# datastax/jvector

Measured on AMD Instinct MI355X. Metric: QPS@recall10>=0.95 (10Mx768); distances/sec as % HBM roofline, higher is better.
Workload: dtype f32

## Files before the change

### jvector_amd/csrc/cabi.cpp

```cpp
#include <algorithm>
#include <cmath>
#include <cstring>
#include <mutex>

#include "jv_device.h"
#include "jv_internal.h"
#include "gs_params.h"
#include "../../include/jvector_formats.h"

namespace jv {

static thread_local char g_err[1024] = "";

void set_error(const char *fmt, ...)
{
    va_list ap;
    va_start(ap, fmt);
    vsnprintf(g_err, sizeof(g_err), fmt, ap);
    va_end(ap);
}
void clear_error() { g_err[0] = 0; }

int Buffer::reserve(size_t bytes)
{
// ... 188 lines not shown
    int n = jv_hip_device_count();
    if (n <= 0) {
        set_error("no HIP device visible (libjvector_hip has no CPU fallback)");
        return JV_ERR_NO_DEVICE;
    }
    JV_REQUIRE(device >= 0 && device < n, "ctx_create: device %d out of range [0,%d)", device, n);
    JV_TRY(use_device(device));
    hipDeviceProp_t prop;
    JV_HIP_CHECK(hipGetDeviceProperties(&prop, device));
    if (strncmp(prop.gcnArchName, "gfx950", 6) != 0) {
        set_error("device %d is %s; this library contains gfx950 code objects only", device, prop.gcnArchName);
        return JV_ERR_NO_DEVICE;
    }
    jv_ctx *c = new jv_ctx();
    c->device = device;
    c->num_cus = prop.multiProcessorCount;
    c->lds_per_block = prop.maxSharedMemoryPerMultiProcessor ? (size_t)prop.maxSharedMemoryPerMultiProcessor
                                                             : (size_t)prop.sharedMemPerBlock;
    if (c->lds_per_block > 160 * 1024) c->lds_per_block = 160 * 1024;
    if (stream != JV_STREAM_PRIVATE) {
        c->stream = (hipStream_t)stream;
        c->owns_stream = false;
    } else {
        hipError_t e = hipStreamCreateWithFlags(&c->stream, hipStreamNonBlocking);
        if (e != hipSuccess) {
            set_error("hipStreamCreate failed: %s", hipGetErrorString(e));
            delete c;
            return JV_ERR_HIP;
        }
        c->owns_stream = true;
    }
    c->h_in.pinned_host = true;
    c->h_out.pinned_host = true;
    *out = c;
    return JV_OK;
}

int jv_hip_ctx_destroy(jv_ctx *ctx)
{
    if (!ctx) return JV_OK;
    (void)hipSetDevice(ctx->device);
    (void)hipStreamSynchronize(ctx->stream);
    if (ctx->host_pool && ctx->host_pool_destroy) ctx->host_pool_destroy(ctx->host_pool);
    ctx->h_in.release();
    ctx->h_out.release();
    ctx->d_in.release();
    ctx->d_out.release();
    ctx->d_scratch.release();
    ctx->d_scratch2.release();
    ctx->d_scratch3.release();
    ctx->d_gs_visited.release();
    ctx->d_gs_spill.release();
    ctx->d_gs_out.release();
    ctx->d_gs_mask.release();
    ctx->d_gs_big.release();
    ctx->d_nvq_q.release();
    ctx->d_gs_extra.release();
    ctx->d_gs_ubr.release();
    ctx->d_bq_work.release();
    ctx->d_bin_work.release();
    ctx->d_bin_cand.release();
    ctx->d_rd_counts.release();
    for (auto &e : ctx->prof_pending) {
        (void)hipEventDestroy(e.start);
        (void)hipEventDestroy(e.stop);
    }
    for (auto &e : ctx->prof_free) (void)hipEventDestroy(e);
    if (ctx->owns_stream) (void)hipStreamDestroy(ctx->stream);
    delete ctx;
    return JV_OK;
}

int jv_hip_ctx_sync(jv_ctx *ctx)
{
    JV_REQUIRE(ctx, "ctx is NULL");
    JV_HIP_CHECK(hipStreamSynchronize(ctx->stream));
    return JV_OK;
}
// ... 615 lines not shown
    l->device = ctx->device;
    l->pq = pq;
    l->capacity = max_queries;
    auto fail = [&](hipError_t e) {
        set_error("luts_create: hipMalloc failed: %s", hipGetErrorString(e));
        (void)hipGetLastError();
        jv_hip_luts_destroy(l);
        return JV_ERR_OOM;
    };
    hipError_t e;
    if ((e = hipMalloc((void **)&l->d_luts, sizeof(float) * (size_t)max_queries * pq->M * kClusters)) != hipSuccess) return fail(e);
    if ((e = hipMalloc((void **)&l->d_bmag, sizeof(float) * (size_t)max_queries)) != hipSuccess) return fail(e);
    if ((e = hipMalloc((void **)&l->d_queries, sizeof(float) * (size_t)max_queries * pq->D)) != hipSuccess) return fail(e);
    if ((e = hipMalloc((void **)&l->d_raw_queries, sizeof(float) * (size_t)max_queries * pq->D)) != hipSuccess) return fail(e);
    *out = l;
    return JV_OK;
}

int jv_hip_luts_destroy(jv_luts *l)
{
    if (!l) return JV_OK;
    (void)hipSetDevice(l->device);
    (void)hipFree(l->d_luts);
    (void)hipFree(l->d_bmag);
    (void)hipFree(l->d_queries);
    (void)hipFree(l->d_raw_queries);
    delete l;
    return JV_OK;
}

}

namespace jv {
int luts_prepare(jv_ctx *ctx, jv_luts *l, const float *queries, int Q, jv_vsf vsf, jv_decoder_kind kind, bool with_tables)
{
    JV_REQUIRE(ctx && l, "luts_build: NULL argument");
    JV_REQUIRE(Q >= 0 && Q <= l->capacity, "luts_build: Q=%d exceeds capacity %d", Q, l->capacity);
    JV_REQUIRE(vsf == JV_EUCLIDEAN || vsf == JV_DOT_PRODUCT || vsf == JV_COSINE, "Unsupported similarity function %d",
               (int)vsf);
    l->Q = Q;
    l->vsf = vsf;
    l->kind = kind;
    l->tables_valid = false;
    if (Q == 0) return JV_OK;
    JV_REQUIRE(queries, "luts_build: queries is NULL");
    JV_TRY(use_device(ctx->device));
    const jv_pq *pq = l->pq;
    const size_t qbytes = sizeof(float) * (size_t)Q * pq->D;
    if (is_device_ptr(queries)) {
        JV_HIP_CHECK(hipMemcpyAsync(l->d_raw_queries, queries, qbytes, hipMemcpyDeviceToDevice, ctx->stream));
    } else {
        JV_HIP_CHECK(hipStreamSynchronize(ctx->stream));
        JV_TRY(ctx->h_in.reserve(qbytes));
        memcpy(ctx->h_in.ptr, queries, qbytes);
        JV_HIP_CHECK(hipMemcpyAsync(l->d_raw_queries, ctx->h_in.ptr, qbytes, hipMemcpyHostToDevice, ctx->stream));
    }
    ProfScope ps(ctx, R_LUT);
    JV_TRY(launch_center_queries(ctx->stream, pq, l->d_raw_queries, Q, l->d_queries));
    if (with_tables) {
        const int lut_vsf = (vsf == JV_EUCLIDEAN) ? VSF_L2 : VSF_DOT;
        JV_TRY(launch_lut_build(ctx->stream, pq, l->d_queries, Q, lut_vsf, l->d_luts));
        l->tables_valid = true;
    }
    if (vsf == JV_COSINE)
        JV_TRY(launch_query_magnitudes(ctx->stream, pq, l->d_queries, Q, kind == JV_DECODER_FUSED ? 1 : 0, l->d_bmag));
    return JV_OK;
}
}

extern "C" {

int jv_hip_luts_build(jv_ctx *ctx, jv_luts *l, const float *queries, int Q, jv_vsf vsf, jv_decoder_kind kind)
{
    clear_error();
    return luts_prepare(ctx, l, queries, Q, vsf, kind, true);
}

int jv_hip_luts_download(jv_ctx *ctx, const jv_luts *l, int q, float *lut_out, float *bmag_out)
{
    clear_error();
    JV_REQUIRE(ctx && l, "luts_download: NULL argument");
    JV_REQUIRE(q >= 0 && q < l->Q, "luts_download: query %d out of range", q);
    JV_REQUIRE(l->tables_valid || !lut_out, "luts_download: the tables were overwritten by a table-free graph search; call jv_hip_luts_build again");
    JV_TRY(use_device(ctx->device));
    JV_HIP_CHECK(hipStreamSynchronize(ctx->stream));
    const size_t n = (size_t)l->pq->M * kClusters;
    if (lut_out) JV_HIP_CHECK(hipMemcpy(lut_out, l->d_luts + (size_t)q * n, sizeof(float) * n, hipMemcpyDefault));
    if (bmag_out) {
        if (l->vsf == JV_COSINE) JV_HIP_CHECK(hipMemcpy(bmag_out, l->d_bmag + q, sizeof(float), hipMemcpyDefault));
        else *bmag_out = 0.0f;
    }
// ... 264 lines not shown
    JV_TRY(ctx->d_scratch.reserve(topk_scratch_bytes(Q, k)));
    OutStage oi, osc;
    JV_TRY(stage_out_begin(ctx, out_ids, sizeof(int32_t) * (size_t)Q * k, ctx->d_out, &oi));
    JV_TRY(stage_out_begin(ctx, out_scores, sizeof(float) * (size_t)Q * k, ctx->d_scratch3, &osc));
    {
        ProfScope ps(ctx, R_TOPK);
        JV_TRY(launch_topk(ctx->stream, ctx, (const float *)d_scores, (const int32_t *)d_ids, Q, n, stride, id_base, k,
                           (int32_t *)oi.dev, (float *)osc.dev, ctx->d_scratch.ptr));
    }
    JV_TRY(stage_out_end(ctx, oi));
    return stage_out_end(ctx, osc);
}

static int next_pow2_i64(int64_t v)
{
    int64_t p = 1;
    while (p < v) p <<= 1;
    return (int)p;
}

int jv_hip_search_flat(jv_ctx *ctx, jv_luts *l, const jv_codes *codes, const jv_vectors *vectors, const float *queries,
                       int Q, jv_vsf vsf, int topK, int rerankK, int32_t id_base, int32_t *out_ids, float *out_scores)
{
    clear_error();
    JV_REQUIRE(ctx && l && codes, "search_flat: NULL argument");
    JV_REQUIRE(topK > 0, "search_flat: topK must be positive");
    const bool rerank = vectors != nullptr && rerankK > 0;
    JV_REQUIRE(!rerank || rerankK >= topK, "rerankK %d must be >= topK %d", rerankK, topK);
    JV_REQUIRE(!rerank || vectors->D == l->pq->D, "search_flat: vector dimension mismatch");
    JV_REQUIRE(!rerank || vectors->count >= codes->count, "search_flat: fewer vectors than codes");
    if (Q == 0) return JV_OK;
    JV_REQUIRE(out_ids && out_scores, "search_flat: NULL output");
    JV_TRY(use_device(ctx->device));
    JV_TRY(jv_hip_luts_build(ctx, l, queries, Q, vsf, JV_DECODER_PQ));
    if (vsf == JV_COSINE) JV_TRY(ensure_code_norms(ctx, const_cast<jv_codes *>(codes)));
    const int64_t N = codes->count;
    const int kvsf = to_kernel_vsf(vsf);
    const int k1 = rerank ? rerankK : topK;

    OutStage oi, osc;
    JV_TRY(stage_out_begin(ctx, out_ids, sizeof(int32_t) * (size_t)Q * topK, ctx->d_out, &oi));
    JV_TRY(stage_out_begin(ctx, out_scores, sizeof(float) * (size_t)Q * topK, ctx->d_in, &osc));

    const size_t c1 = (size_t)Q * k1;
    JV_TRY(ctx->d_scratch3.reserve(sizeof(int32_t) * c1 + sizeof(float) * c1 * 2 + sizeof(float) * (size_t)Q + 1024));
    int32_t *d_cand = (int32_t *)ctx->d_scratch3.ptr;
    float *d_cand_sc = (float *)(d_cand + c1);
    float *d_exact = d_cand_sc + c1;
    float *d_qnorm = d_exact + c1;
    int32_t *d_k1_ids = rerank ? d_cand : (int32_t *)oi.dev;
    float *d_k1_sc = rerank ? d_cand_sc : (float *)osc.dev;

    bool done1 = false;
    const bool mq = adc_mq_supported(codes->M, codes->d_codes) && Q >= 2;
    if (mq && N >= (1 << 18) && (int64_t)k1 * 64 <= N && ctx_opt(ctx, "no_filter", 0) == 0) {
        const int64_t c_target = std::max<int64_t>(3 * (int64_t)k1, 4096);
        int64_t S_target = std::max<int64_t>(16384, next_pow2_i64(32 * N / c_target));
        const int64_t stride = std::max<int64_t>(1, N / S_target);
        const int64_t S = N / stride;
        const int k_s = (int)std::max<int64_t>(16, (c_target * S + N - 1) / N);
        const int cap = (int)std::min<int64_t>(N, 4 * c_target);
        if (k_s <= 4096 && S >= k_s) {
            const size_t b_samp = sizeof(float) * (size_t)Q * S, b_ks = sizeof(float) * (size_t)Q * k_s;
            const size_t b_cap = sizeof(float) * (size_t)Q * cap;
            JV_TRY(ctx->d_scratch2.reserve(b_samp + 2 * b_ks + 2 * b_cap + sizeof(unsigned int) * (size_t)Q + 1024));
            char *base = (char *)ctx->d_scratch2.ptr;
            float *d_samp = (float *)base;
// ... 67 lines not shown
            JV_HIP_CHECK(hipMemcpyAsync(ctx->h_out.ptr, d_cnt, sizeof(unsigned int) * (size_t)Q, hipMemcpyDeviceToHost,
                                        ctx->stream));
            JV_HIP_CHECK(hipStreamSynchronize(ctx->stream));
            const unsigned int *cnt = (const unsigned int *)ctx->h_out.ptr;
            bool ok = true;
            for (int q = 0; q < Q; ++q) ok = ok && cnt[q] >= (unsigned int)k1 && cnt[q] <= (unsigned int)cap;
            if (ok) {
                ProfScope ps(ctx, R_TOPK);
                JV_TRY(launch_topk(ctx->stream, ctx, d_f_sc, d_f_ids, Q, cap, cap, 0, k1, d_k1_ids, d_k1_sc,
                                   ctx->d_scratch.ptr, d_cnt));
                done1 = true;
            }
            }
        }
    }
    if (!done1) {
        JV_TRY(ctx->d_scratch2.reserve(sizeof(float) * (size_t)Q * N));
        float *d_scores = (float *)ctx->d_scratch2.ptr;
        JV_TRY(ctx->d_scratch.reserve(topk_scratch_bytes(Q, std::max(k1, topK))));
        {
            ProfScope ps(ctx, R_ADC);
            if (mq)
                JV_TRY(launch_adc_mq_store(ctx->stream, ctx, l->d_luts, l->d_bmag, Q, codes->M, kvsf, codes->d_codes,
                                           codes->d_norms, 0, N, 1, d_scores));
            else
                JV_TRY(launch_adc(ctx->stream, ctx, l->d_luts, l->d_bmag, Q, codes->M, kvsf, codes->d_codes,
                                  codes->d_norms, N, 0, N, nullptr, d_scores));
        }
        ProfScope ps(ctx, R_TOPK);
        JV_TRY(launch_topk(ctx->stream, ctx, d_scores, nullptr, Q, N, N, 0, k1, d_k1_ids, d_k1_sc, ctx->d_scratch.ptr));
    }

    if (rerank) {
        JV_TRY(rerank_gather(ctx, vectors, l->d_raw_queries, Q, vsf, d_cand, k1, d_exact, d_qnorm));
        ProfScope ps(ctx, R_TOPK);
        JV_TRY(launch_topk(ctx->stream, ctx, d_exact, d_cand, Q, k1, k1, 0, topK, (int32_t *)oi.dev, (float *)osc.dev,
                           ctx->d_scratch.ptr));
    }
    JV_TRY(launch_add_id_base(ctx->stream, (int32_t *)oi.dev, (int64_t)Q * topK, id_base));
    JV_TRY(stage_out_end(ctx, oi));
    return stage_out_end(ctx, osc);
}

}
```

### jvector_amd/csrc/graph_search.cpp

```cpp
#include <algorithm>
#include <atomic>
#include <chrono>
#include <condition_variable>
#include <cstdlib>
#include <functional>
#include <memory>
#include <unordered_map>
#include <mutex>
#include <thread>

#include "gs_host.h"
#include "gs_params.h"
#include "jv_internal.h"

namespace jv {
constexpr long long kGsUbrDefault = 1;
constexpr long long kGsUbrcDefault = 1;


class HostPool {
public:
    explicit HostPool(int nthreads) : n_(nthreads)
    {
        for (int t = 1; t < n_; ++t) threads_.emplace_back([this, t] { worker(t); });
// ... 1161 lines not shown
    out->max_degree = 0;
    for (int l = 0; l <= g->entry_level; ++l) {
        const jv_graph::DevLevel &d = g->dev[l];
        lv[l].nbrs = d.nbrs;
        lv[l].hkeys = d.hkeys;
        lv[l].hvals = d.hvals;
        lv[l].hmask = d.hmask;
        lv[l].hshift = d.hshift;
        lv[l].count = g->levels[l].count;
        lv[l].degree = g->levels[l].degree;
        out->max_degree = std::max(out->max_degree, g->levels[l].degree);
    }
    return JV_OK;
}
}
}

struct DeviceSessionOut {
    float threshold = 0.0f;
    const std::vector<jv_searcher::Call> *history = nullptr;
    int new_rerankK = 0;
    int log_cap = 0;
    std::vector<int32_t> status, base, log_n;
    std::vector<int64_t> stats;
    std::vector<long long> log;
};

static int graph_search_device(jv_ctx *ctx, const jv_graph *g, jv_luts *l, const jv_codes *codes, const jv_fused *fused,
                               const jv_vectors *vectors, const float *queries, int Q, jv_vsf vsf, int topK, int rerankK,
                               int32_t *out_ids, float *out_scores, int64_t *stats, AcceptMask host_accept, AcceptMask dev_accept,
                               DeviceSessionOut *so = nullptr)
{
    const jv_decoder_kind kind = fused ? JV_DECODER_FUSED : JV_DECODER_PQ;
    JV_TRY(luts_prepare(ctx, l, queries, Q, vsf, kind, false));
    const int kvsf = to_kernel_vsf(vsf);
    if (vsf == JV_COSINE) {
        JV_TRY(ensure_code_norms(ctx, const_cast<jv_codes *>(codes)));
        if (fused) JV_TRY(ensure_fused_norms(ctx, const_cast<jv_fused *>(fused)));
    }
    JV_TRY(ensure_device_graph(ctx, const_cast<jv_graph *>(g)));
    const jv_pq *pq = l->pq;

    const bool generic = !graph_search_device_specialised(pq, codes, fused) || ctx_opt(ctx, "gs_generic", 0) != 0;
    const int occ = ctx_opt(ctx, "gs_occ", generic ? 4 : 2) >= 4 ? 4 : 2;
    bool pair = occ == 2 && !generic && ctx_opt(ctx, "gs_pair", 1) != 0;
    for (int lv = 0; lv <= g->entry_level; ++lv) pair = pair && g->levels[lv].degree <= 32;
    pair = pair && pq->M <= 96;
    const long long wgx_opt = ctx_opt(ctx, "gs_wgx", -1);
    bool one_wave_tuned = false;
    for (const char *o : {"gs_vcap_log2", "gs_v1_log2", "gs_grow", "gs_retry", "gs_occ", "gs_pair", "gs_cand_cap", "gs_waves_per_cu", "gs_prefetch", "gs_prof"})
        one_wave_tuned = one_wave_tuned || ctx_opt_is_set(ctx, o);
    bool wgx = !so && !generic && graph_search_wgx_supported(pq->M) &&
               (wgx_opt > 0 || (wgx_opt < 0 && !one_wave_tuned && Q <= 4 * ctx->num_cus));
    for (int lv = 0; lv <= g->entry_level; ++lv) wgx = wgx && g->levels[lv].degree <= 64;
    const int wgx_log = std::min(512, std::max(256, 4 * rerankK));
    int wgx_kps = 32;
    for (int lv = 0; lv <= g->entry_level; ++lv)
        if (g->levels[lv].degree > 32) wgx_kps = 64;
    const int wgx_waves = std::max(2, std::min(8, (int)ctx_opt(ctx, "gs_wgx_waves", 8)));
    const int wgx_slots = std::max(2, std::min((int)GX_MAX_SLOTS, (int)ctx_opt(ctx, "gs_wgx_slots", 16)));
    int evict_cap = GS_EVICT_CAP;
    const int wgx_cand_cap = 256;
    const int wgx_per_cu = std::max(1, std::min(4, (int)ctx_opt(ctx, "gs_wgx_per_cu", 1)));
    const size_t wgx_budget = ctx->lds_per_block / (size_t)wgx_per_cu - (wgx_per_cu > 1 ? 256 : 512);
    auto wgx_bytes = [&](int lg, int lm) { return graph_search_wgx_lds_bytes(pq->D, rerankK, wgx_cand_cap, evict_cap, lg, wgx_slots, wgx_kps, wgx_log, lm); };
    int wgx_lut_m = (int)ctx_opt(ctx, "gs_wgx_lut_m", 0);
    if (wgx) {
// ... 233 lines not shown
        p.big_visited = (int32_t *)ctx->d_gs_big.ptr;
        p.big_spill = (long long *)((char *)ctx->d_gs_big.ptr + big_spill_off);
        p.big_next = (uint32_t *)((char *)ctx->d_gs_big.ptr + big_ctr_off);
        p.big_count = big_count;
        p.big_log2 = big_log2;
        p.big_spill_cap = big_spill_cap;
    }
    p.pair = pair ? 1 : (pairc ? 2 : 0);
#ifdef JV_EXPERIMENTAL
    p.quad = ctx_opt(ctx, "gs_quad", 0) != 0 ? 1 : 0;
#else
    p.quad = 0;
#endif
    p.out_ids = d_cand;
    p.out_scores = d_cand_sc;
    p.out_stats = d_stats;
    p.out_status = d_status;
    p.next_query = d_counter;
    if (log_cap > 0) {
        p.push_log = (long long *)(base + o_log);
        p.push_log_n = (int32_t *)(base + o_log_n);
        p.push_log_cap = log_cap;
    }
    p.prof = gs_prof ? (unsigned long long *)(base + o_prof) : nullptr;
    p.plain = ctx_opt(ctx, "gs_plain", 1) != 0 ? 1 : 0;
    if (defer_on) {
        p.defer = 1;
        p.defer_count = (unsigned long long *)(base + o_prof) + 33;
        p.defer_min_level = (int)std::max<long long>(1, ctx_opt(ctx, "gs_defer_min_level", 2));
    }
    int rr_rows = 0;
    if (!so && !wgx && ubr && pair && vectors && !vectors->nvq && vectors->D == pq->D && gs_rr_lds_bytes() <= lds && ctx_opt(ctx, "gs_fused_rerank", 1) != 0) {
        if (vsf == JV_COSINE) JV_TRY(ensure_vector_norms(ctx, const_cast<jv_vectors *>(vectors)));
        rr_rows = exact_fused_rows(vectors->d_vecs, vectors->D, l->d_raw_queries, Q, kvsf, rerankK, vectors->d_sqnorm);
    }
    if (rr_rows > 0) {
        if (vsf == JV_COSINE) {
            ProfScope ps(ctx, R_EXACT);
            JV_TRY(launch_query_sqnorms(ctx->stream, l->d_raw_queries, vectors->D, Q, d_qnorm));
        }
        p.rr_vecs = vectors->d_vecs;
        p.rr_queries = l->d_raw_queries;
        p.rr_qnorm = d_qnorm;
        p.rr_vnorm = vectors->d_sqnorm;
        p.rr_n = vectors->count;
        p.rr_rows = rr_rows;
    }
    {
        ProfScope ps(ctx, R_GSEARCH);
        JV_TRY(launch(p, workers));
    }
    std::vector<int32_t> status((size_t)Q);
    std::vector<int> redo;
    size_t n_overflow_first = 0;
    {
        JV_TRY(ctx->h_out.reserve(sizeof(int32_t) * (size_t)Q));
        JV_HIP_CHECK(hipMemcpyAsync(ctx->h_out.ptr, d_status, sizeof(int32_t) * (size_t)Q, hipMemcpyDeviceToHost, ctx->stream));
        unsigned long long ubr_dropped = 0;
        if (ubr) JV_HIP_CHECK(hipMemcpyAsync(&ubr_dropped, base + o_prof + 15 * sizeof(unsigned long long), sizeof(ubr_dropped), hipMemcpyDeviceToHost, ctx->stream));
        unsigned long long defer_counts[3] = {0, 0, 0};
        if (defer_on) JV_HIP_CHECK(hipMemcpyAsync(defer_counts, base + o_prof + 33 * sizeof(unsigned long long), sizeof(defer_counts), hipMemcpyDeviceToHost, ctx->stream));
        JV_HIP_CHECK(hipStreamSynchronize(ctx->stream));
        if (ubr) ctx_stat_add(ctx, "gs_ubr_dropped", (long long)ubr_dropped);
        if (defer_on) {
            ctx_stat_add(ctx, "gs_deferred", (long long)defer_counts[0]);
            ctx_stat_add(ctx, "gs_defer_restarts", (long long)defer_counts[1]);
            if (Q >= 64 && defer_counts[1] * 10 > (unsigned long long)Q && g->defer_off.exchange(1, std::memory_order_relaxed) == 0)
                ctx_stat_add(ctx, "gs_defer_switched_off", 1);
        }
        memcpy(status.data(), ctx->h_out.ptr, sizeof(int32_t) * (size_t)Q);
        for (int q = 0; q < Q; ++q)
            if (status[q] != GS_OK) redo.push_back(q);
        n_overflow_first = redo.size();
    }
    const bool retry = ctx_opt_is_set(ctx, "gs_retry") ? ctx_opt(ctx, "gs_retry", 1) != 0 : !ctx_opt_is_set(ctx, "gs_vcap_log2");
    for (int attempt = 1; attempt <= 2 && !redo.empty() && retry; ++attempt) {
        const int vlog2 = std::min(24, vcap_log2 + 3 * attempt);
        if (vlog2 <= vcap_log2 + 3 * (attempt - 1)) break;
        const size_t vcap2 = (size_t)1 << vlog2;
        const int spill2 = (int)(vcap2 / 2 + v1_slots) + 64;
        const int R = (int)redo.size();
        const int workers2 = std::max(1, std::min<int>({R, workers, (int)(((size_t)512 << 20) / (vcap2 * 12))}));
        JV_TRY(ctx->d_gs_visited.reserve(sizeof(int32_t) * vcap2 * (size_t)workers2));
        JV_TRY(ctx->d_gs_spill.reserve(sizeof(long long) * (size_t)spill2 * (size_t)workers2));
        memcpy(ctx->h_out.ptr, redo.data(), sizeof(int32_t) * (size_t)R);
        JV_HIP_CHECK(hipMemcpyAsync(base + o_qmap, ctx->h_out.ptr, sizeof(int32_t) * (size_t)R, hipMemcpyHostToDevice, ctx->stream));
        JV_HIP_CHECK(hipMemsetAsync(d_counter, 0, sizeof(uint32_t), ctx->stream));
        GsParams p2 = p;
        p2.qmap = (const int32_t *)(base + o_qmap);
        p2.Q = R;
        p2.visited = (int32_t *)ctx->d_gs_visited.ptr;
        p2.vcap_log2 = vlog2;
        p2.spill = (long long *)ctx->d_gs_spill.ptr;
        p2.spill_cap = spill2;
        p2.big_visited = nullptr;
        p2.big_count = 0;
        p2.big_log2 = 0;
        p2.prof = nullptr;
        p2.defer = 0;
        {
            ProfScope ps(ctx, R_GSEARCH);
            JV_TRY(launch(p2, workers2));
        }
        JV_HIP_CHECK(hipStreamSynchronize(ctx->stream));
        JV_HIP_CHECK(hipMemcpyAsync(ctx->h_out.ptr, d_status, sizeof(int32_t) * (size_t)Q, hipMemcpyDeviceToHost, ctx->stream));
        JV_HIP_CHECK(hipStreamSynchronize(ctx->stream));
        memcpy(status.data(), ctx->h_out.ptr, sizeof(int32_t) * (size_t)Q);
        std::vector<int> still;
        for (int q : redo)
            if (status[q] != GS_OK) still.push_back(q);
        redo.swap(still);
    }
    if (gs_prof) {
        unsigned long long h[33];
        JV_HIP_CHECK(hipMemcpyAsync(h, base + o_prof, sizeof(h), hipMemcpyDeviceToHost, ctx->stream));
        JV_HIP_CHECK(hipStreamSynchronize(ctx->stream));
        const double e = (double)std::max<unsigned long long>(h[5], 1);
        fprintf(stderr, "[jv gs prof] clocks/expansion: pop %.0f  result %.0f  row+block+visited %.0f  score %.0f  push %.0f | expansions %llu "
                        "queries %llu  setup+epilogue clocks/query %.0f\n", h[0] / e, h[1] / e, h[2] / e, h[3] / e, h[4] / e, h[5], h[6],
                (double)h[7] / (double)std::max<unsigned long long>(h[6], 1));
        const double fs = (double)std::max<unsigned long long>(h[8] + h[9] + h[10] + h[11], 1);
        {
            const double nq = (double)std::max<unsigned long long>(h[6], 1);
            fprintf(stderr, "[jv gs prof] clocks/query outside the expansion loop: setup %.0f  level transitions %.0f  epilogue %.0f  table build %.0f\n",
                    h[12] / nq, h[13] / nq, h[14] / nq, h[15] / nq);
            fprintf(stderr, "[jv gs prof] levels above 0: %.2f expansions per query, %.0f clocks per query (searchOneLayer + transitions) = %.0f per expansion\n",
                    h[24] / nq, h[25] / nq, (double)h[25] / (double)std::max<unsigned long long>(h[24], 1));
            {
                const double eu = (double)std::max<unsigned long long>(h[24], 1);
                fprintf(stderr, "[jv gs prof] levels above 0, clocks/expansion: pop %.0f  result %.0f  row+visited %.0f  score %.0f  push %.0f | scoring passes %.2f per expansion, %.0f clocks per pass\n",
                        h[26] / eu, h[27] / eu, h[28] / eu, h[29] / eu, h[30] / eu, h[32] / eu, (double)h[31] / (double)std::max<unsigned long long>(h[32], 1));
            }
        }
        if (wgx)
            fprintf(stderr, "[jv gs prof] workgroup form, per expansion: row found in a slot %.3f (of those still being scored at use: %.3f of all)  "
                            "requested at the pop %.3f  rows requested ahead %.3f\n", h[8] / e, h[9] / e, h[10] / e, h[11] / e);
        else if (ubr) {
            fprintf(stderr, "[jv gs prof] register-table bound form, per expansion: bound + staging %.0f clocks  bound + staging + exact scores %.0f clocks  "
                            "trims %.0f clocks | dropped %.2f  exactly scored %.2f neighbours\n", h[8] / e, h[9] / e, h[10] / e, h[15] / e, h[11] / e);
            fprintf(stderr, "[jv gs prof] register-table bound form, per expansion: wait for the row %.0f clocks  scoring rounds %.0f  owner sum + finish %.0f  "
                            "passes %.2f | expansions with <= 4 / <= 8 / <= 16 survivors: %.3f / %.3f / %.3f\n", h[16] / e, h[17] / e, h[18] / e, h[19] / e,
                    h[20] / e, h[21] / e, h[22] / e);
        }
        else
        fprintf(stderr, "[jv gs prof] scored neighbours by fresh count of their expansion: <=8 %.3f  <=16 %.3f  <=24 %.3f  <=32 %.3f\n", h[8] / fs,
                h[9] / fs, h[10] / fs, h[11] / fs);
    }

    if (so) {
        so->status.assign(status.begin(), status.end());
        so->base.resize((size_t)Q);
        so->log_n.resize((size_t)Q);
        so->stats.resize(2 * (size_t)Q);
        JV_HIP_CHECK(hipMemcpyAsync(so->base.data(), base + o_base, sizeof(int32_t) * (size_t)Q, hipMemcpyDeviceToHost, ctx->stream));
        JV_HIP_CHECK(hipMemcpyAsync(so->log_n.data(), base + o_log_n, sizeof(int32_t) * (size_t)Q, hipMemcpyDeviceToHost, ctx->stream));
        JV_HIP_CHECK(hipMemcpyAsync(so->stats.data(), d_stats, sizeof(long long) * 2 * (size_t)Q, hipMemcpyDeviceToHost, ctx->stream));
        JV_HIP_CHECK(hipStreamSynchronize(ctx->stream));
        int longest = 0;
        bool overflowed = false;
        for (int q = 0; q < Q; ++q) {
            overflowed = overflowed || so->log_n[(size_t)q] > log_cap;
            longest = std::max(longest, std::min(so->log_n[(size_t)q], log_cap));
        }
        so->log_cap = overflowed ? -1 : std::max(longest, 1);
        if (!overflowed) {
            so->log.resize((size_t)Q * (size_t)so->log_cap);
            JV_HIP_CHECK(hipMemcpy2DAsync(so->log.data(), sizeof(long long) * (size_t)so->log_cap, base + o_log, sizeof(long long) * (size_t)log_cap,
                                          sizeof(long long) * (size_t)so->log_cap, (size_t)Q, hipMemcpyDeviceToHost, ctx->stream));
            JV_HIP_CHECK(hipStreamSynchronize(ctx->stream));
        }
        ctx_stat_add(ctx, "gs_calls_device", 1);
        ctx_stat_add(ctx, "gs_queries_device", Q);
        ctx_stat_add(ctx, "gs_session_calls_device", 1);
        return JV_OK;
    }
    OutStage oi, osc;
    JV_TRY(stage_out_begin(ctx, out_ids, sizeof(int32_t) * (size_t)Q * topK, ctx->d_scratch2, &oi));
    JV_TRY(stage_out_begin(ctx, out_scores, sizeof(float) * (size_t)Q * topK, ctx->d_scratch3, &osc));
    JV_TRY(ctx->d_scratch.reserve(topk_scratch_bytes(Q, topK)));
    if (vectors && rr_rows > 0) {
        if (rr_rows < rerankK) {
            ProfScope ps(ctx, R_EXACT);
            JV_TRY(launch_exact_gather_tail(ctx->stream, vectors->d_vecs, vectors->count, vectors->D, l->d_raw_queries, Q, kvsf, d_cand, rerankK, rr_rows,
                                            d_cand_sc, d_qnorm, vectors->d_sqnorm));
        }
    } else if (vectors) {
        JV_TRY(rerank_gather(ctx, vectors, l->d_raw_queries, Q, vsf, d_cand, rerankK, d_cand_sc, d_qnorm));
    }
    {
        ProfScope ps(ctx, R_TOPK);
        JV_TRY(launch_topk(ctx->stream, ctx, d_cand_sc, d_cand, Q, rerankK, rerankK, 0, topK, (int32_t *)oi.dev,
                           (float *)osc.dev, ctx->d_scratch.ptr));
    }
    if (tie_check) {
        JV_HIP_CHECK(hipMemsetAsync(d_counter, 0, sizeof(uint32_t) * 2, ctx->stream));
        ProfScope ps(ctx, R_TOPK);
        RtParams rt{};
        rt.cand_sc = d_cand_sc;
        rt.cand_ids = d_cand;
        rt.R = rerankK;
        rt.out_sc = (float *)osc.dev;
        rt.out_ids = (int32_t *)oi.dev;
        rt.K = topK;
        rt.Q = Q;
        rt.push_log = p.push_log;
        rt.push_log_n = p.push_log_n;
        rt.log_cap = p.push_log_cap;
        rt.rerankK = rerankK;
        rt.status = d_status;
        rt.count = d_counter;
        JV_TRY(launch_rerank_ties(ctx->stream, rt));
    }
    JV_TRY(stage_out_end(ctx, oi));
    JV_TRY(stage_out_end(ctx, osc));
    const size_t stats_bytes = stats ? sizeof(long long) * 2 * (size_t)Q : 0;
    JV_TRY(ctx->h_out.reserve(stats_bytes + 64));
    unsigned int *h_ties = (unsigned int *)((char *)ctx->h_out.ptr + stats_bytes);
    h_ties[0] = h_ties[1] = 0;
    if (tie_check) JV_HIP_CHECK(hipMemcpyAsync(h_ties, d_counter, sizeof(uint32_t) * 2, hipMemcpyDeviceToHost, ctx->stream));
    if (stats) {
        long long *h_stats = (long long *)ctx->h_out.ptr;
        JV_HIP_CHECK(hipMemcpyAsync(h_stats, d_stats, sizeof(long long) * 2 * (size_t)Q, hipMemcpyDeviceToHost, ctx->stream));
        JV_HIP_CHECK(hipStreamSynchronize(ctx->stream));
        for (int q = 0; q < Q; ++q) {
            stats[2 * q] = h_stats[2 * q];
            stats[2 * q + 1] = h_stats[2 * q + 1];
        }
    } else {
        JV_HIP_CHECK(hipStreamSynchronize(ctx->stream));
    }
    const size_t n_ties = h_ties[0], n_ties_resolved = h_ties[1];
    if (n_ties > 0) {
        JV_TRY(ctx->h_out.reserve(sizeof(int32_t) * (size_t)Q));
        JV_HIP_CHECK(hipMemcpyAsync(ctx->h_out.ptr, d_status, sizeof(int32_t) * (size_t)Q, hipMemcpyDeviceToHost, ctx->stream));
        JV_HIP_CHECK(hipStreamSynchronize(ctx->stream));
        const int32_t *hs = (const int32_t *)ctx->h_out.ptr;
        for (int q = 0; q < Q; ++q)
            if (hs[q] == GS_RERANK_TIE) redo.push_back(q);
        std::sort(redo.begin(), redo.end());
    }
    ctx_stat_add(ctx, "gs_calls_device", 1);
    ctx_stat_add(ctx, "gs_queries_device", Q);
    ctx_stat_add(ctx, "gs_queries_retried", (long long)n_overflow_first);
    ctx_stat_add(ctx, "gs_ties_resolved_device", (long long)n_ties_resolved);
    ctx_stat_add(ctx, "gs_ties_to_host", (long long)n_ties);
    ctx_stat_add(ctx, "gs_queries_host_fallback", (long long)redo.size());
    ctx_stat_set(ctx, "gs_last_v1_log2", v1_log2);
    ctx_stat_set(ctx, "gs_last_workers_per_cu", per_cu);
    ctx_stat_set(ctx, "gs_last_wgx", wgx ? 1 : 0);
    ctx_stat_set(ctx, "gs_last_ubr", ubr ? 1 : 0);
    ctx_stat_set(ctx, "gs_last_plain", (!wgx && gs_params_plain(p)) ? 1 : 0);
    ctx_stat_set(ctx, "gs_last_rr_rows", rr_rows);
    ctx_stat_set(ctx, "gs_last_pair", pair ? 1 : (pairc ? 2 : 0));
    if (wgx) ctx_stat_add(ctx, "gs_calls_wgx", 1);
    if (ctx_opt(ctx, "graph_timing", 0) != 0)
        fprintf(stderr, "[jv graph_search device] Q=%d workers=%d (x%d/CU, occ %d, pair %d, wgx %d) lds=%zu cand_cap=%d evict_cap=%d v1_log2=%d vcap=%zu overflow=%zu rerank ties=%zu (+%zu to the host) -> host %zu\n", Q,
                workers, per_cu, occ, pair ? 1 : (pairc ? 2 : 0), wgx ? wgx_waves : 0, lds, cand_cap, evict_cap, v1_log2, vcap, n_overflow_first, n_ties_resolved, n_ties, redo.size());
    if (redo.empty()) return JV_OK;

    jv_graph *gm = const_cast<jv_graph *>(g);
    std::unique_lock<std::mutex> loan_lock(gm->dev_mu, std::defer_lock);
    if (g->dev_level0) loan_lock.lock();
    struct Level0Loan {
        jv_graph *g;
        bool active = false;
        ~Level0Loan()
        {
            if (active) {
                g->levels[0].nbrs.clear();
                g->levels[0].nbrs.shrink_to_fit();
            }
// ... 474 lines not shown
```

### jvector_amd/csrc/jv_internal.h

```cpp
#pragma once

#include <hip/hip_runtime.h>

#include <algorithm>
#include <atomic>
#include <cmath>
#include <cstdarg>
#include <cstdint>
#include <cstdio>
#include <cstring>
#include <string>
#include <map>
#include <string>
#include <vector>

#include "../../include/jvector_hip.h"

namespace jv {

constexpr int kClusters = 256;
constexpr int kMaxGraphDegree = 512;

void set_error(const char *fmt, ...);
void clear_error();
// ... 31 lines not shown
    } while (0)

struct Buffer {
    void *ptr = nullptr;
    size_t cap = 0;
    bool pinned_host = false;
    int reserve(size_t bytes);
    void release();
};

}

namespace jv {
enum Region : int { R_ADC = 0, R_TOPK, R_EXACT, R_LUT, R_ENCODE, R_NORMS, R_SAMPLE, R_GSEARCH, R_PRUNE, R_ADC_EXACT, R_COUNT };
struct ProfEvent {
    int region;
    hipEvent_t start, stop;
};
}

struct jv_ctx {
    bool profiling = false;
    std::vector<jv::ProfEvent> prof_pending;
    std::vector<hipEvent_t> prof_free;
    double prof_ms[jv::R_COUNT] = {0};
    int64_t prof_count[jv::R_COUNT] = {0};
    int device = 0;
    hipStream_t stream = nullptr;
    bool owns_stream = false;
    int num_cus = 256;
    size_t lds_per_block = 65536;
    jv::Buffer h_in, h_out, d_in, d_out, d_scratch, d_scratch2, d_scratch3;
    jv::Buffer d_gs_visited, d_gs_spill, d_gs_out, d_gs_mask, d_gs_big;
    jv::Buffer d_gs_extra;
    jv::Buffer d_gs_ubr;
    jv::Buffer d_bq_work;
    jv::Buffer d_bin_work, d_bin_cand;
    jv::Buffer d_rd_counts;
    jv::Buffer d_nvq_q;
    void *host_pool = nullptr;
    void (*host_pool_destroy)(void *) = nullptr;
    std::atomic<int> busy{0};
    std::map<std::string, long long> opts, stats;
};

namespace jv {
inline uint64_t next_fused_generation()
{
    static std::atomic<uint64_t> g{1};
    return g.fetch_add(1, std::memory_order_relaxed);
}
long long ctx_opt(const jv_ctx *ctx, const char *name, long long dflt);
bool ctx_opt_is_set(const jv_ctx *ctx, const char *name);
inline void ctx_stat_add(jv_ctx *ctx, const char *name, long long v) { ctx->stats[name] += v; }
inline void ctx_stat_set(jv_ctx *ctx, const char *name, long long v) { ctx->stats[name] = v; }

struct CtxBusy {
    jv_ctx *c;
    bool ok;
    explicit CtxBusy(jv_ctx *cc) : c(cc), ok(cc->busy.exchange(1, std::memory_order_acquire) == 0) {}
    ~CtxBusy()
    {
        if (ok) c->busy.store(0, std::memory_order_release);
    }
};
}
// ... 59 lines not shown

struct jv_pair_table {
    int device = 0;
    const jv_pq *pq = nullptr;
    jv_vsf vsf = JV_EUCLIDEAN;
    float *d_tri = nullptr;
    int64_t floats = 0;
    float *d_sq = nullptr;
};

struct jv_fused {
    int device = 0;
    const jv_pq *pq = nullptr;
    int64_t count = 0;
    int maxDegree = 0, M = 0;
    uint8_t *d_blocks = nullptr;
    int32_t *d_neighbors = nullptr;
    float *d_norms = nullptr;
    bool norms_valid = false;
    uint64_t generation = 0;
};

struct jv_luts {
    int device = 0;
    const jv_pq *pq = nullptr;
    int capacity = 0;
    int Q = 0;
    jv_vsf vsf = JV_EUCLIDEAN;
    jv_decoder_kind kind = JV_DECODER_PQ;
    float *d_luts = nullptr;
    float *d_bmag = nullptr;
    float *d_queries = nullptr;
    float *d_raw_queries = nullptr;
    bool tables_valid = false;
};

struct jv_layered {
    int device = 0, max_degree = 0;
    int64_t n = 0;
    int32_t entry = -1;
    int entry_level = 0;
    std::vector<std::vector<int32_t>> nodes;
    std::vector<std::vector<int32_t>> nbrs;
    int32_t *d_level0 = nullptr;
    double seconds[3] = {0, 0, 0}, total_s = 0;
    int64_t counts[5] = {0, 0, 0, 0, 0};
    std::vector<int64_t> level_counts;
};

namespace jv {
inline uint64_t splitmix64(uint64_t &s)
{
    uint64_t z = (s += 0x9E3779B97F4A7C15ull);
    z = (z ^ (z >> 30)) * 0xBF58476D1CE4E5B9ull;
    z = (z ^ (z >> 27)) * 0x94D049BB133111EBull;
    return z ^ (z >> 31);
}
inline std::vector<int32_t> seeded_permutation(int64_t n, uint64_t seed)
{
    std::vector<int32_t> p((size_t)n);
    for (int64_t i = 0; i < n; ++i) p[(size_t)i] = (int32_t)i;
    uint64_t st = seed;
    for (int64_t i = n - 1; i > 0; --i) {
        const int64_t j = (int64_t)(splitmix64(st) % (uint64_t)(i + 1));
        std::swap(p[(size_t)i], p[(size_t)j]);
    }
// ... 158 lines not shown
int launch_bl_ro_apply_selection(hipStream_t s, const BlRoApplyParams &p);
int launch_bl_ro_backlink_merge(hipStream_t s, const BlRoMergeParams &p);
int launch_bl_ro_rewrite_rows(hipStream_t s, const BlRoRowsParams &p);
int launch_bl_ro_copy_rows(hipStream_t s, const BlRoCopyParams &p);
struct BlRoImproveParams;
struct BlSelIdsParams;
struct BlRoApplySortedParams;
int launch_bl_sel_ids(hipStream_t s, const BlSelIdsParams &p);
int launch_bl_ro_apply_sorted(hipStream_t s, const BlRoApplySortedParams &p);
struct BlRoRowEdgesParams;
int launch_bl_ro_improve_list(hipStream_t s, const BlRoImproveParams &p);
int launch_bl_ro_row_edges(hipStream_t s, const BlRoRowEdgesParams &p);
int launch_bl_apply_selection(hipStream_t s, const BlApplyParams &p);
int launch_bl_backlink_merge(hipStream_t s, const BlMergeParams &p);
int launch_bl_improve_list(hipStream_t s, const BlImproveParams &p);
int launch_bl_row_edges(hipStream_t s, const BlRowEdgesParams &p);
int launch_bl_rank_sort(hipStream_t s, const BlSortParams &p);
int launch_bl_rewrite_rows(hipStream_t s, const BlRowsParams &p);
int launch_bl_list_over_degree(hipStream_t s, const BlOverParams &p);
int launch_bl_count_valid(hipStream_t s, const int32_t *cand, int C, int32_t *count, long long B);
int launch_bl_copy_rows(hipStream_t s, const int32_t *nbrs, int R, const int32_t *tgt, long long P, int32_t *out);
int launch_bl_strided_copy(hipStream_t s, const int32_t *src, int R, int Rf, long long N, int32_t *dst);
int launch_bl_sort_edges(hipStream_t s, void *temp, size_t *temp_bytes, const unsigned long long *keys_in, unsigned long long *keys_out,
                         const int32_t *vals_in, int32_t *vals_out, long long n, int end_bit);
struct GsParams;
struct GsLevel;
struct GraphDeviceView {
    int64_t n_nodes = 0;
    int32_t entry_node = -1;
    int entry_level = 0;
    int max_degree = 0;
};
int graph_device_view(jv_ctx *ctx, const jv_graph *g, GsLevel *lv, GraphDeviceView *out);
int luts_prepare(jv_ctx *ctx, jv_luts *l, const float *queries, int Q, jv_vsf vsf, jv_decoder_kind kind, bool with_tables);
int pq_create_impl(jv_ctx *ctx, int D, int M, int k, const int *sizes, const float *codebooks, const float *centroid, bool pad, jv_pq **out);
bool graph_search_device_supported(const jv_pq *pq, const jv_codes *codes, const jv_fused *fused, int max_degree, int n_levels);
bool graph_search_device_specialised(const jv_pq *pq, const jv_codes *codes, const jv_fused *fused);
size_t graph_search_lds_bytes(int D, int rerankK, int cand_cap, int pair_M, int evict_cap = 0, int v1_log2 = 0);
int launch_graph_search(hipStream_t s, int vsf, const GsParams &p, int workers, int occupancy);
bool graph_search_ubr_supported(int M, int kernel_vsf);
int launch_ubr_tables(hipStream_t s, int vsf, const float *codebooks, const float *cq, int Q, int M, uint32_t *tab, float *meta);
int launch_graph_search_ubr(hipStream_t s, int vsf, const GsParams &p, int workers, size_t lds);
bool graph_search_wgx_supported(int M);
size_t graph_search_wgx_lds_bytes(int D, int rerankK, int cand_cap, int evict_cap, int v1_log2, int slots, int kps, int logcap, int M);
int launch_graph_search_wgx(hipStream_t s, int vsf, const GsParams &p, int workgroups, int threads);
bool graph_search_session_supported(int M);
int launch_graph_search_session(hipStream_t s, int vsf, const GsParams &p, int workers, size_t lds);
size_t topk_scratch_bytes(int Q, int k);
struct RtParams;
int launch_rerank_ties(hipStream_t s, const RtParams &p);
int launch_topk(hipStream_t s, const jv_ctx *ctx, const float *d_scores, const int32_t *d_ids, int Q, int64_t n,
                int64_t stride, int32_t id_base, int k, int32_t *d_out_ids, float *d_out_scores, void *d_scratch,
                const unsigned int *d_row_counts = nullptr);
bool adc_mq_supported(int M, const uint8_t *d_codes);
int launch_adc_mq_store(hipStream_t s, const jv_ctx *ctx, const float *d_luts, const float *d_bmag, int Q, int M,
                        int vsf, const uint8_t *d_codes, const float *d_norms, int64_t first, int64_t count,
                        int64_t row_stride, float *d_out);
int launch_adc_mq_filter(hipStream_t s, const jv_ctx *ctx, const float *d_luts, const float *d_bmag, int Q, int M,
                         int vsf, const uint8_t *d_codes, const float *d_norms, int64_t first, int64_t count,
                         const float *d_tau, int tau_stride, int32_t *d_cand_ids, float *d_cand_scores,
                         unsigned int *d_cand_count, int cap);
bool adc_bq_supported(int M, const uint8_t *d_codes, size_t lds_per_block);
size_t adc_bq_scratch_bytes(int Q, int M);
int launch_adc_bq_scan(hipStream_t s, const jv_ctx *ctx, const float *d_luts, const float *d_bmag, int Q, int M, int vsf, const uint8_t *d_codes,
                       const float *d_norms, int64_t first, int64_t count, const float *d_tau, int tau_stride, int32_t *d_ids,
                       unsigned int *d_surv_cnt, int cap2, void *d_work);
int launch_adc_bq_exact(hipStream_t s, const jv_ctx *ctx, const float *d_luts, const float *d_bmag, int Q, int M, int vsf, const uint8_t *d_codes,
// ... 8 lines not shown
```

Before: 2.592 million.

## Defer graph-search status readback past rerank and borrow device query buffers

The host no longer synchronises right after the graph search kernel to read per-query overflow status. Status is now copied into a pinned buffer and checked after the rerank/top-k stage. Retries only rerun the finishing stage when some query actually overflowed. Device-resident queries that are suitably aligned are used in place instead of being copied device-to-device. This removes one stream sync and one copy per batch, at the price of redoing rerank/top-k work when retries occur and more complex control flow.

```diff
diff --git a/jvector_amd/csrc/cabi.cpp b/jvector_amd/csrc/cabi.cpp
--- a/jvector_amd/csrc/cabi.cpp
+++ b/jvector_amd/csrc/cabi.cpp
@@ -244,6 +244,7 @@
     }
     c->h_in.pinned_host = true;
     c->h_out.pinned_host = true;
+    c->h_gs_status.pinned_host = true;
     *out = c;
     return JV_OK;
 }
@@ -256,6 +257,7 @@
     if (ctx->host_pool && ctx->host_pool_destroy) ctx->host_pool_destroy(ctx->host_pool);
     ctx->h_in.release();
     ctx->h_out.release();
+    ctx->h_gs_status.release();
     ctx->d_in.release();
     ctx->d_out.release();
     ctx->d_scratch.release();
@@ -937,7 +939,7 @@
 }
 
 namespace jv {
-int luts_prepare(jv_ctx *ctx, jv_luts *l, const float *queries, int Q, jv_vsf vsf, jv_decoder_kind kind, bool with_tables)
+int luts_prepare(jv_ctx *ctx, jv_luts *l, const float *queries, int Q, jv_vsf vsf, jv_decoder_kind kind, bool with_tables, bool borrow_queries)
 {
     JV_REQUIRE(ctx && l, "luts_build: NULL argument");
     JV_REQUIRE(Q >= 0 && Q <= l->capacity, "luts_build: Q=%d exceeds capacity %d", Q, l->capacity);
@@ -947,13 +949,15 @@
     l->vsf = vsf;
     l->kind = kind;
     l->tables_valid = false;
+    l->d_raw_view = l->d_raw_queries;
     if (Q == 0) return JV_OK;
     JV_REQUIRE(queries, "luts_build: queries is NULL");
     JV_TRY(use_device(ctx->device));
     const jv_pq *pq = l->pq;
     const size_t qbytes = sizeof(float) * (size_t)Q * pq->D;
     if (is_device_ptr(queries)) {
-        JV_HIP_CHECK(hipMemcpyAsync(l->d_raw_queries, queries, qbytes, hipMemcpyDeviceToDevice, ctx->stream));
+        if (borrow_queries && pq->D % 8 == 0 && pq->D >= 8 && (reinterpret_cast<uintptr_t>(queries) & 15) == 0) l->d_raw_view = queries;
+        else JV_HIP_CHECK(hipMemcpyAsync(l->d_raw_queries, queries, qbytes, hipMemcpyDeviceToDevice, ctx->stream));
     } else {
         JV_HIP_CHECK(hipStreamSynchronize(ctx->stream));
         JV_TRY(ctx->h_in.reserve(qbytes));
@@ -961,7 +965,7 @@
         JV_HIP_CHECK(hipMemcpyAsync(l->d_raw_queries, ctx->h_in.ptr, qbytes, hipMemcpyHostToDevice, ctx->stream));
     }
     ProfScope ps(ctx, R_LUT);
-    JV_TRY(launch_center_queries(ctx->stream, pq, l->d_raw_queries, Q, l->d_queries));
+    JV_TRY(launch_center_queries(ctx->stream, pq, l->d_raw_view, Q, l->d_queries));
     if (with_tables) {
         const int lut_vsf = (vsf == JV_EUCLIDEAN) ? VSF_L2 : VSF_DOT;
         JV_TRY(launch_lut_build(ctx->stream, pq, l->d_queries, Q, lut_vsf, l->d_luts));
@@ -1292,7 +1296,7 @@
     if (Q == 0) return JV_OK;
     JV_REQUIRE(out_ids && out_scores, "search_flat: NULL output");
     JV_TRY(use_device(ctx->device));
-    JV_TRY(jv_hip_luts_build(ctx, l, queries, Q, vsf, JV_DECODER_PQ));
+    JV_TRY(luts_prepare(ctx, l, queries, Q, vsf, JV_DECODER_PQ, true, !is_device_ptr(out_ids) || !is_device_ptr(out_scores)));
     if (vsf == JV_COSINE) JV_TRY(ensure_code_norms(ctx, const_cast<jv_codes *>(codes)));
     const int64_t N = codes->count;
     const int kvsf = to_kernel_vsf(vsf);
@@ -1426,7 +1430,7 @@
     }
 
     if (rerank) {
-        JV_TRY(rerank_gather(ctx, vectors, l->d_raw_queries, Q, vsf, d_cand, k1, d_exact, d_qnorm));
+        JV_TRY(rerank_gather(ctx, vectors, l->d_raw_view, Q, vsf, d_cand, k1, d_exact, d_qnorm));
         ProfScope ps(ctx, R_TOPK);
         JV_TRY(launch_topk(ctx->stream, ctx, d_exact, d_cand, Q, k1, k1, 0, topK, (int32_t *)oi.dev, (float *)osc.dev,
                            ctx->d_scratch.ptr));
diff --git a/jvector_amd/csrc/graph_search.cpp b/jvector_amd/csrc/graph_search.cpp
--- a/jvector_amd/csrc/graph_search.cpp
+++ b/jvector_amd/csrc/graph_search.cpp
@@ -1217,7 +1217,7 @@
                                DeviceSessionOut *so = nullptr)
 {
     const jv_decoder_kind kind = fused ? JV_DECODER_FUSED : JV_DECODER_PQ;
-    JV_TRY(luts_prepare(ctx, l, queries, Q, vsf, kind, false));
+    JV_TRY(luts_prepare(ctx, l, queries, Q, vsf, kind, false, so == nullptr));
     const int kvsf = to_kernel_vsf(vsf);
     if (vsf == JV_COSINE) {
         JV_TRY(ensure_code_norms(ctx, const_cast<jv_codes *>(codes)));
@@ -1517,15 +1517,15 @@
     int rr_rows = 0;
     if (!so && !wgx && ubr && pair && vectors && !vectors->nvq && vectors->D == pq->D && gs_rr_lds_bytes() <= lds && ctx_opt(ctx, "gs_fused_rerank", 1) != 0) {
         if (vsf == JV_COSINE) JV_TRY(ensure_vector_norms(ctx, const_cast<jv_vectors *>(vectors)));
-        rr_rows = exact_fused_rows(vectors->d_vecs, vectors->D, l->d_raw_queries, Q, kvsf, rerankK, vectors->d_sqnorm);
+        rr_rows = exact_fused_rows(vectors->d_vecs, vectors->D, l->d_raw_view, Q, kvsf, rerankK, vectors->d_sqnorm);
     }
     if (rr_rows > 0) {
         if (vsf == JV_COSINE) {
             ProfScope ps(ctx, R_EXACT);
-            JV_TRY(launch_query_sqnorms(ctx->stream, l->d_raw_queries, vectors->D, Q, d_qnorm));
+            JV_TRY(launch_query_sqnorms(ctx->stream, l->d_raw_view, vectors->D, Q, d_qnorm));
         }
         p.rr_vecs = vectors->d_vecs;
-        p.rr_queries = l->d_raw_queries;
+        p.rr_queries = l->d_raw_view;
         p.rr_qnorm = d_qnorm;
         p.rr_vnorm = vectors->d_sqnorm;
         p.rr_n = vectors->count;
@@ -1535,30 +1535,32 @@
         ProfScope ps(ctx, R_GSEARCH);
         JV_TRY(launch(p, workers));
     }
-    std::vector<int32_t> status((size_t)Q);
+    const bool retry = ctx_opt_is_set(ctx, "gs_retry") ? ctx_opt(ctx, "gs_retry", 1) != 0 : !ctx_opt_is_set(ctx, "gs_vcap_log2");
+    const bool early_status = so || gs_prof || (ctx_opt_is_set(ctx, "gs_vcap_log2") && !retry);
+    const size_t status_bytes = (sizeof(int32_t) * (size_t)Q + 15) & ~(size_t)15;
+    JV_TRY(ctx->h_gs_status.reserve(2 * status_bytes + 4 * sizeof(unsigned long long)));
+    int32_t *status = (int32_t *)ctx->h_gs_status.ptr;
+    int32_t *status_now = (int32_t *)((char *)ctx->h_gs_status.ptr + status_bytes);
+    unsigned long long *h_counts = (unsigned long long *)((char *)ctx->h_gs_status.ptr + 2 * status_bytes);
     std::vector<int> redo;
     size_t n_overflow_first = 0;
-    {
-        JV_TRY(ctx->h_out.reserve(sizeof(int32_t) * (size_t)Q));
-        JV_HIP_CHECK(hipMemcpyAsync(ctx->h_out.ptr, d_status, sizeof(int32_t) * (size_t)Q, hipMemcpyDeviceToHost, ctx->stream));
-        unsigned long long ubr_dropped = 0;
-        if (ubr) JV_HIP_CHECK(hipMemcpyAsync(&ubr_dropped, base + o_prof + 15 * sizeof(unsigned long long), sizeof(ubr_dropped), hipMemcpyDeviceToHost, ctx->stream));
-        unsigned long long defer_counts[3] = {0, 0, 0};
-        if (defer_on) JV_HIP_CHECK(hipMemcpyAsync(defer_counts, base + o_prof + 33 * sizeof(unsigned long long), sizeof(defer_counts), hipMemcpyDeviceToHost, ctx->stream));
-        JV_HIP_CHECK(hipStreamSynchronize(ctx->stream));
-        if (ubr) ctx_stat_add(ctx, "gs_ubr_dropped", (long long)ubr_dropped);
+    h_counts[0] = h_counts[1] = h_counts[2] = h_counts[3] = 0;
+    JV_HIP_CHECK(hipMemcpyAsync(status, d_status, sizeof(int32_t) * (size_t)Q, hipMemcpyDeviceToHost, ctx->stream));
+    if (ubr) JV_HIP_CHECK(hipMemcpyAsync(h_counts, base + o_prof + 15 * sizeof(unsigned long long), sizeof(unsigned long long), hipMemcpyDeviceToHost, ctx->stream));
+    if (defer_on) JV_HIP_CHECK(hipMemcpyAsync(h_counts + 1, base + o_prof + 33 * sizeof(unsigned long long), 3 * sizeof(unsigned long long), hipMemcpyDeviceToHost, ctx->stream));
+    auto read_status = [&]() {
+        if (ubr) ctx_stat_add(ctx, "gs_ubr_dropped", (long long)h_counts[0]);
         if (defer_on) {
-            ctx_stat_add(ctx, "gs_deferred", (long long)defer_counts[0]);
-            ctx_stat_add(ctx, "gs_defer_restarts", (long long)defer_counts[1]);
-            if (Q >= 64 && defer_counts[1] * 10 > (unsigned long long)Q && g->defer_off.exchange(1, std::memory_order_relaxed) == 0)
+            ctx_stat_add(ctx, "gs_deferred", (long long)h_counts[1]);
+            ctx_stat_add(ctx, "gs_defer_restarts", (long long)h_counts[2]);
+            if (Q >= 64 && h_counts[2] * 10 > (unsigned long long)Q && g->defer_off.exchange(1, std::memory_order_relaxed) == 0)
                 ctx_stat_add(ctx, "gs_defer_switched_off", 1);
         }
-        memcpy(status.data(), ctx->h_out.ptr, sizeof(int32_t) * (size_t)Q);
         for (int q = 0; q < Q; ++q)
             if (status[q] != GS_OK) redo.push_back(q);
         n_overflow_first = redo.size();
-    }
-    const bool retry = ctx_opt_is_set(ctx, "gs_retry") ? ctx_opt(ctx, "gs_retry", 1) != 0 : !ctx_opt_is_set(ctx, "gs_vcap_log2");
+    };
+    auto retry_passes = [&]() -> int {
     for (int attempt = 1; attempt <= 2 && !redo.empty() && retry; ++attempt) {
         const int vlog2 = std::min(24, vcap_log2 + 3 * attempt);
         if (vlog2 <= vcap_log2 + 3 * (attempt - 1)) break;
@@ -1568,8 +1570,8 @@
         const int workers2 = std::max(1, std::min<int>({R, workers, (int)(((size_t)512 << 20) / (vcap2 * 12))}));
         JV_TRY(ctx->d_gs_visited.reserve(sizeof(int32_t) * vcap2 * (size_t)workers2));
         JV_TRY(ctx->d_gs_spill.reserve(sizeof(long long) * (size_t)spill2 * (size_t)workers2));
-        memcpy(ctx->h_out.ptr, redo.data(), sizeof(int32_t) * (size_t)R);
-        JV_HIP_CHECK(hipMemcpyAsync(base + o_qmap, ctx->h_out.ptr, sizeof(int32_t) * (size_t)R, hipMemcpyHostToDevice, ctx->stream));
+        memcpy(status_now, redo.data(), sizeof(int32_t) * (size_t)R);
+        JV_HIP_CHECK(hipMemcpyAsync(base + o_qmap, status_now, sizeof(int32_t) * (size_t)R, hipMemcpyHostToDevice, ctx->stream));
         JV_HIP_CHECK(hipMemsetAsync(d_counter, 0, sizeof(uint32_t), ctx->stream));
         GsParams p2 = p;
         p2.qmap = (const int32_t *)(base + o_qmap);
@@ -1588,13 +1590,21 @@
             JV_TRY(launch(p2, workers2));
         }
         JV_HIP_CHECK(hipStreamSynchronize(ctx->stream));
-        JV_HIP_CHECK(hipMemcpyAsync(ctx->h_out.ptr, d_status, sizeof(int32_t) * (size_t)Q, hipMemcpyDeviceToHost, ctx->stream));
+        JV_HIP_CHECK(hipMemcpyAsync(status_now, d_status, sizeof(int32_t) * (size_t)Q, hipMemcpyDeviceToHost, ctx->stream));
         JV_HIP_CHECK(hipStreamSynchronize(ctx->stream));
-        memcpy(status.data(), ctx->h_out.ptr, sizeof(int32_t) * (size_t)Q);
         std::vector<int> still;
-        for (int q : redo)
+        for (int q : redo) {
+            status[q] = status_now[q];
             if (status[q] != GS_OK) still.push_back(q);
+        }
         redo.swap(still);
+    }
+    return JV_OK;
+    };
+    if (early_status) {
+        JV_HIP_CHECK(hipStreamSynchronize(ctx->stream));
+        read_status();
+        JV_TRY(retry_passes());
     }
     if (gs_prof) {
         unsigned long long h[33];
@@ -1633,7 +1643,7 @@
     }
 
     if (so) {
-        so->status.assign(status.begin(), status.end());
+        so->status.assign(status, status + Q);
         so->base.resize((size_t)Q);
         so->log_n.resize((size_t)Q);
         so->stats.resize(2 * (size_t)Q);
@@ -1663,14 +1673,17 @@
     JV_TRY(stage_out_begin(ctx, out_ids, sizeof(int32_t) * (size_t)Q * topK, ctx->d_scratch2, &oi));
     JV_TRY(stage_out_begin(ctx, out_scores, sizeof(float) * (size_t)Q * topK, ctx->d_scratch3, &osc));
     JV_TRY(ctx->d_scratch.reserve(topk_scratch_bytes(Q, topK)));
+    size_t n_ties = 0, n_ties_resolved = 0;
+    std::vector<int> tie_redo;
+    auto finish_batch = [&]() -> int {
     if (vectors && rr_rows > 0) {
         if (rr_rows < rerankK) {
             ProfScope ps(ctx, R_EXACT);
-            JV_TRY(launch_exact_gather_tail(ctx->stream, vectors->d_vecs, vectors->count, vectors->D, l->d_raw_queries, Q, kvsf, d_cand, rerankK, rr_rows,
+            JV_TRY(launch_exact_gather_tail(ctx->stream, vectors->d_vecs, vectors->count, vectors->D, l->d_raw_view, Q, kvsf, d_cand, rerankK, rr_rows,
                                             d_cand_sc, d_qnorm, vectors->d_sqnorm));
         }
     } else if (vectors) {
-        JV_TRY(rerank_gather(ctx, vectors, l->d_raw_queries, Q, vsf, d_cand, rerankK, d_cand_sc, d_qnorm));
+        JV_TRY(rerank_gather(ctx, vectors, l->d_raw_view, Q, vsf, d_cand, rerankK, d_cand_sc, d_qnorm));
     }
     {
         ProfScope ps(ctx, R_TOPK);
@@ -1714,14 +1727,30 @@
     } else {
         JV_HIP_CHECK(hipStreamSynchronize(ctx->stream));
     }
-    const size_t n_ties = h_ties[0], n_ties_resolved = h_ties[1];
+    n_ties = h_ties[0];
+    n_ties_resolved = h_ties[1];
+    tie_redo.clear();
     if (n_ties > 0) {
         JV_TRY(ctx->h_out.reserve(sizeof(int32_t) * (size_t)Q));
         JV_HIP_CHECK(hipMemcpyAsync(ctx->h_out.ptr, d_status, sizeof(int32_t) * (size_t)Q, hipMemcpyDeviceToHost, ctx->stream));
         JV_HIP_CHECK(hipStreamSynchronize(ctx->stream));
         const int32_t *hs = (const int32_t *)ctx->h_out.ptr;
         for (int q = 0; q < Q; ++q)
-            if (hs[q] == GS_RERANK_TIE) redo.push_back(q);
+            if (hs[q] == GS_RERANK_TIE) tie_redo.push_back(q);
+    }
+    return JV_OK;
+    };
+    JV_TRY(finish_batch());
+    if (!early_status) {
+        read_status();
+        if (!redo.empty() && retry) {
+            JV_TRY(retry_passes());
+            JV_HIP_CHECK(hipMemcpyAsync(d_status, status, sizeof(int32_t) * (size_t)Q, hipMemcpyHostToDevice, ctx->stream));
+            JV_TRY(finish_batch());
+        }
+    }
+    if (!tie_redo.empty()) {
+        redo.insert(redo.end(), tie_redo.begin(), tie_redo.end());
         std::sort(redo.begin(), redo.end());
     }
     ctx_stat_add(ctx, "gs_calls_device", 1);
diff --git a/jvector_amd/csrc/jv_internal.h b/jvector_amd/csrc/jv_internal.h
--- a/jvector_amd/csrc/jv_internal.h
+++ b/jvector_amd/csrc/jv_internal.h
@@ -87,6 +87,7 @@
     size_t lds_per_block = 65536;
     jv::Buffer h_in, h_out, d_in, d_out, d_scratch, d_scratch2, d_scratch3;
     jv::Buffer d_gs_visited, d_gs_spill, d_gs_out, d_gs_mask, d_gs_big;
+    jv::Buffer h_gs_status;
     jv::Buffer d_gs_extra;
     jv::Buffer d_gs_ubr;
     jv::Buffer d_bq_work;
@@ -212,6 +213,7 @@
     float *d_bmag = nullptr;
     float *d_queries = nullptr;
     float *d_raw_queries = nullptr;
+    const float *d_raw_view = nullptr;
     bool tables_valid = false;
 };
 
@@ -436,7 +438,7 @@
     int max_degree = 0;
 };
 int graph_device_view(jv_ctx *ctx, const jv_graph *g, GsLevel *lv, GraphDeviceView *out);
-int luts_prepare(jv_ctx *ctx, jv_luts *l, const float *queries, int Q, jv_vsf vsf, jv_decoder_kind kind, bool with_tables);
+int luts_prepare(jv_ctx *ctx, jv_luts *l, const float *queries, int Q, jv_vsf vsf, jv_decoder_kind kind, bool with_tables, bool borrow_queries = false);
 int pq_create_impl(jv_ctx *ctx, int D, int M, int k, const int *sizes, const float *codebooks, const float *centroid, bool pad, jv_pq **out);
 bool graph_search_device_supported(const jv_pq *pq, const jv_codes *codes, const jv_fused *fused, int max_degree, int n_levels);
 bool graph_search_device_specialised(const jv_pq *pq, const jv_codes *codes, const jv_fused *fused);
```

Result: no change. 2.603 million (median of 6 runs) (+0.4%).
